# zju3dv/neuralbody

Hardware: NVIDIA H100
Metric: rays_per_s_512x512_64spp (higher is better)
Workload: dtype f16x2 (hi+lo fp16 pairs, fp32 accumulate)

## Files before the change

neuralbody_b200/csrc/nb_render_tc_list.cu:

```cuda
#include "nb_tc_common.cuh"
#include <type_traits>

namespace nb {
namespace tcl {

using tcr::Quad;

constexpr int TP = 128;
constexpr int NUM_SEGS = 6;
constexpr int MAXS = 1024;
constexpr uint32_t ID_MASK = 0x0FFFFFFFu;

__device__ __forceinline__ unsigned long long global_ns() {
    unsigned long long t;
    asm volatile("mov.u64 %0, %%globaltimer;" : "=l"(t));
    return t;
}

__device__ __forceinline__ void load_frame_xf(const RenderParams& P, FrameXf* xf, int i) {
    const int b = P.frame;
    if (i < 9) xf->R[i] = __ldg(P.R + b * 9 + i);
    if (i < 3) {
        xf->Th[i] = __ldg(P.Th + b * 3 + i);
        xf->min_dhw[i] = __ldg(P.bounds + b * 6 + (2 - i));
        xf->voxel[i] = P.voxel_size[i];
        xf->out_sh[i] = P.out_sh[i];
    }
}

constexpr int CLS_THREADS = 256, CLS_PER_THREAD = MAXS / CLS_THREADS;
__global__ void __launch_bounds__(CLS_THREADS) classify_compact_kernel(const __grid_constant__ RenderParams P) {
    __shared__ FrameXf xf;
// ... 69 lines not shown
    for (int k = 0; k < CLS_PER_THREAD; ++k) {
        const int slot = k * (CLS_THREADS / 32) + warp;
        const int c = cls[k];
        const uint32_t same = __match_any_sync(0xffffffffu, c);
        if (c >= 0) {
            int local = __popc(same & ((1u << lane) - 1));
            for (int w = 0; w < slot; ++w) local += wcnt[c][w];
            float4* buf = c >= 2 ? P.list_a : P.list_b;
            const size_t at = (c & 1) ? (size_t)sbase[c] + local : P.list_cap - (size_t)sbase[c] - stotal[c] + local;
            buf[at] = gm[k];
        } else if (live[k]) {
            P.raw_ws[(__float_as_uint(gm[k].w) & ID_MASK) - id0] = empty;
        }
    }
}

constexpr int NT = 384;
constexpr int NROWT = 96;
constexpr int LAUNCH_REGS = (65536 / NT) / 8 * 8;
constexpr int PRODUCER_REGS = 56, CONSUMER_REGS = 224;
constexpr int CHUNK_STRIDE = TP * 16 + 16;
constexpr int ACT_CHUNKS = kHidden / 8;
constexpr int PLANE_BYTES = ACT_CHUNKS * CHUNK_STRIDE;
constexpr int SEG_BUFS = 4;
constexpr int SLOT_BYTES = 16384, NUM_SLOTS = 4;
constexpr int TILE256 = kHalfTile256 * 2;
constexpr int TILE3 = kHalfTile3 * 2;
constexpr int L3_PUSH = 4;
constexpr int L3_PUSHES = (kStepsL3 + L3_PUSH - 1) / L3_PUSH;
constexpr int HEAD_FLOATS = kHidden + 4 + 3 * kColor + 4 + 3 * kHidden;
constexpr int H_ALPHA = 0, H_RGBW = kHidden + 4, H_RGBB = H_RGBW + 3 * kColor, H_B0 = H_RGBB + 4;
constexpr int OFF_HI = 0, OFF_LO = PLANE_BYTES;
constexpr int OFF_RING = 2 * PLANE_BYTES;
constexpr int OFF_HEAD = OFF_RING + NUM_SLOTS * SLOT_BYTES;
constexpr int OFF_XF = OFF_HEAD + HEAD_FLOATS * 4;
constexpr int OFF_SCHED = OFF_XF + 128;
constexpr int OFF_ROWS = OFF_SCHED + 64;
constexpr int NV_COARSE = 64, NV_FINE = 128;
__host__ __device__ constexpr int level_nv(int li) { return li < 2 ? NV_COARSE : NV_FINE; }
__host__ __device__ constexpr int level_channels(int li) { return li < 2 ? 128 : li == 2 ? 64 : 32; }
__host__ __device__ constexpr int ids_at(int li, int half) {
    return li < 2 ? (2 * li + half) * NV_COARSE : 4 * NV_COARSE + (2 * (li - 2) + half) * NV_FINE;
}
constexpr int HBITS = 8, HSIZE = 1 << HBITS;
constexpr uint32_t HEMPTY = 0xFFFFFFFFu;
struct VoxTable {
    float4 grid[TP];
// ... 266 lines not shown
                    auto put = [&](int k, float v) {
                        const __half hv = __float2half_rn(v);
                        asm volatile("st.shared.b16 [%0], %1;" ::"r"(s_lo + act_off(prow, k)), "h"(*reinterpret_cast<const unsigned short*>(&hv)) : "memory");
                    };
                    if (job < TP) {
                        positional_embed_anchored<10, 5>(e.x, e.y, e.z, [&](int j, float v) { put(j, v); });
                        put(63, 0.f);
                    } else {
                        const int smp = (int)(__float_as_uint(e.w) & ID_MASK);
                        const size_t ri = (size_t)P.frame * P.n_rays + (prow < nrows ? smp / S : 0);
                        const float dx = __ldg(P.ray_d + ri * 3), dy = __ldg(P.ray_d + ri * 3 + 1), dz = __ldg(P.ray_d + ri * 3 + 2);
                        const float nrm = sqrtf(__fadd_rn(__fadd_rn(__fmul_rn(dx, dx), __fmul_rn(dy, dy)), __fmul_rn(dz, dz)));
                        positional_embed_anchored<4, 4>(__fdiv_rn(dx, nrm), __fdiv_rn(dy, nrm), __fdiv_rn(dz, nrm), [&](int j, float v) { put(64 + j, v); });
                        put(91, 0.f); put(92, 1.f); put(93, 1.f); put(94, 0.f); put(95, 0.f);
                    }
                }
                tc::fence_proxy_async();
                tc::mbar_arrive(&bars[B_PEFULL]);
                tr.ev(32);
            }
        }
    } else {
        tc::setmaxnreg_inc<CONSUMER_REGS>();
        uint32_t s_hi, s_lo;
        const int cw = wgid - 1;
        const bool arr = lane == 0;
        int tn = ((tid & 127) == 0 && blockIdx.x == 0 && P.trace) ? (1 + cw) * 4096 : -1;
        auto tval = [&](int code, unsigned long long v) {
            if (tn >= 0 && tn < (2 + cw) * 4096) P.trace[tn++] = ((unsigned long long)code << 48) | (v & 0xFFFFFFFFFFFFull);
        };
        auto tev = [&](int code) { tval(code, (unsigned long long)clock64()); };
        const int r0 = 64 * cw + 16 * (warp & 3) + (lane >> 2), cq = 2 * (lane & 3);
        float acc0[64], acc1[64];
        auto init_bias = [&](const float* b) {
#pragma unroll
            for (int c = 0; c < 16; ++c) {
                const float2 v0 = *reinterpret_cast<const float2*>(b + 8 * c + cq), v1 = *reinterpret_cast<const float2*>(b + 128 + 8 * c + cq);
                acc0[4 * c] = v0.x; acc0[4 * c + 1] = v0.y; acc0[4 * c + 2] = v0.x; acc0[4 * c + 3] = v0.y;
                acc1[4 * c] = v1.x; acc1[4 * c + 1] = v1.y; acc1[4 * c + 2] = v1.x; acc1[4 * c + 3] = v1.y;
            }
        };
        const uint32_t wg_rows = (uint32_t)(cw * 8 * 128);
        auto mma256 = [&](uint32_t slot, int ka) {
            const uint64_t a_hi = tc::make_smem_desc(s_hi + wg_rows + 2 * ka * CHUNK_STRIDE, CHUNK_STRIDE, 128);
            const uint64_t a_lo = tc::make_smem_desc(s_lo + wg_rows + 2 * ka * CHUNK_STRIDE, CHUNK_STRIDE, 128);
            const uint64_t b0h = tc::make_smem_desc(slot + 0 * TILE256, 128 * 16, 128);
            const uint64_t b0l = tc::make_smem_desc(slot + 1 * TILE256, 128 * 16, 128);
            const uint64_t b1h = tc::make_smem_desc(slot + 2 * TILE256, 128 * 16, 128);
            const uint64_t b1l = tc::make_smem_desc(slot + 3 * TILE256, 128 * 16, 128);
            tc::wgmma_m64n128k16_f16(acc0, a_hi, b0h, true);
            tc::wgmma_m64n128k16_f16(acc1, a_hi, b1h, true);
            if (NP == 3) {
                tc::wgmma_m64n128k16_f16(acc0, a_lo, b0h, true);
                tc::wgmma_m64n128k16_f16(acc1, a_lo, b1h, true);
                tc::wgmma_m64n128k16_f16(acc0, a_hi, b0l, true);
                tc::wgmma_m64n128k16_f16(acc1, a_hi, b1l, true);
            }
        };
        uint32_t g = 0;
        uint32_t w_stall = 0, r_stall = 0, pe_stall = 0, g_coarse = 0, g_fine = 0;
        auto take = [&](auto&& mma) {
            const uint32_t s = g % NUM_SLOTS;
            const uint32_t t0 = (uint32_t)clock();
            tc::mbar_wait(&bars[B_FULL + s], (g / NUM_SLOTS) & 1);
            w_stall += (uint32_t)clock() - t0;
            tc::wgmma_fence();
            mma(s_ring + s * SLOT_BYTES);
            tc::wgmma_commit();
            ++g;
        };
        auto release = [&](uint32_t gp, bool pred) { tc::mbar_arrive_if(&bars[B_EMPTY + gp % NUM_SLOTS], pred); };
        auto release_last = [&]() { release(g - 1, arr); };

        auto convert = [&](bool last) {
            float sig0 = 0.f, sig1 = 0.f;
            auto one = [&](const float (&a)[64], int nh) {
#pragma unroll
                for (int c = 0; c < 16; ++c) {
                    const int col = 128 * nh + 8 * c + cq;
#pragma unroll
                    for (int hr = 0; hr < 2; ++hr) {
                        const float x0 = a[4 * c + 2 * hr], x1 = a[4 * c + 2 * hr + 1];
                        const uint32_t off = act_off(r0 + 8 * hr, col);
                        uint32_t hv;
                        if (last) {
                            const float2 aw = *reinterpret_cast<const float2*>(head + H_ALPHA + col);
                            float& sg = hr ? sig1 : sig0;
                            sg = fmaf(fmaxf(x0, 0.f), aw.x, sg);
                            sg = fmaf(fmaxf(x1, 0.f), aw.y, sg);
                            hv = tc::cvt_relu_f16x2(x0, x1);
                        } else if (NP == 3) {
                            hv = tc::cvt_rz_relu_f16x2(x0, x1);
                            float q0, q1;
                            tc::trunc_residual2(x0, x1, q0, q1);
                            const uint32_t lv = tc::cvt_relu_f16x2(q0, q1);
                            asm volatile("st.shared.b32 [%0], %1;" ::"r"(s_lo + off), "r"(lv) : "memory");
                        } else {
                            hv = tc::cvt_relu_f16x2(x0, x1);
                        }
                        asm volatile("st.shared.b32 [%0], %1;" ::"r"(s_hi + off), "r"(hv) : "memory");
                    }
                }
            };
            one(acc0, 0);
            one(acc1, 1);
            return make_float2(sig0, sig1);
        };
        auto publish = [&]() {
            tc::fence_proxy_async();
            tcr::named_bar_sync(1 + cw, 128);
        };

        int it = 0;
        for (int tile = blockIdx.x; tile < n_tiles; tile += gridDim.x, ++it) {
            const TileRef tref = tile_ref(tile);
            const int nrows = tref.nrows, nseg = class_segments(tref.cls);
            const float4* rows = rows_buf + (it & 1) * TP;
            asm volatile("mov.u32 %0, %1;" : "=r"(s_hi) : "r"(s_hi0));
            asm volatile("mov.u32 %0, %1;" : "=r"(s_lo) : "r"(s_lo0));
            tev(1);
            auto gather = [&](int seg) {
                const unsigned char* volbase = reinterpret_cast<const unsigned char*>(P.volume);
                const VoxTable* vt = reinterpret_cast<const VoxTable*>(smem + OFF_VTAB) + (it & 1);
                const int grp = (tid & 127) >> 3, t = tid & 7;
                const int lvl = seg < 2 ? 3 : seg < 4 ? 2 : seg < 5 ? 1 : 0;
                const int cbase0 = seg < 2 ? seg * 64 : seg < 4 ? (seg - 2) * 64 : 0;
                const int nunits = seg == NUM_SEGS - 1 ? 1 : 2;
                const int C = P.lvl_C[lvl], D = P.lvl_D[lvl], H = P.lvl_H[lvl], W = P.lvl_W[lvl];
                const int kb = 64 * (seg % SEG_BUFS);
                const int li = seg < 4 ? seg >> 1 : seg - 2;
                const int lg_vb = (li < 2 ? 7 : li == 2 ? 6 : 5) + (sizeof(VT) == 4 ? 2 : 1), lg_vpp = 10 - lg_vb;
                const bool staged = C == level_channels(li) && vt->n[2 * li + cw] <= (uint32_t)level_nv(li);
                const uint32_t st_base = s_hi + (li == 1 ? 0 : 16) * CHUNK_STRIDE + cw * 1024;
                auto stage_addr = [&](uint32_t v) {
                    const uint32_t p = v >> lg_vpp;
                    return st_base + (p >> 4) * PLANE_BYTES + (p & 15) * CHUNK_STRIDE + ((v & ((1u << lg_vpp) - 1)) << lg_vb);
                };
                if (staged && (seg >= 4 || (seg & 1) == 0)) {
                    const unsigned char* src = volbase + P.lvl_off[lvl] + (size_t)P.frame * P.lvl_bstride[lvl] * sizeof(VT);
                    const uint32_t* ids = vt->ids + ids_at(li, cw);
                    const int lg_ppv = lg_vb - 4;
                    const uint32_t nq = vt->n[2 * li + cw] << lg_ppv;
#pragma unroll 4
                    for (uint32_t i = tid & 127; i < nq; i += 128) {
                        const uint32_t v = i >> lg_ppv, q = i & ((1u << lg_ppv) - 1);
                        tc::cp_async_16(stage_addr(v) + 16 * q, src + ((size_t)ids[v] << lg_vb) + 16 * q);
                    }
                    tc::cp_async_wait_all();
                    tcr::named_bar_sync(1 + cw, 128);
                }
                auto setup = [&](float gx, float gy, float gz, float (&cw)[8]) {
                    Corners cn;
                    const uint32_t cb = clamped_cell(gx, gy, gz, W, H, D, cn);
#pragma unroll
                    for (int c = 0; c < 8; ++c) cw[c] = __fmul_rn(__fmul_rn(cn.wx[c & 1], cn.wy[(c >> 1) & 1]), cn.wz[c >> 2]);
                    return cb;
                };
                auto store_row = [&](int row, const float (&acc)[2][4]) {
#pragma unroll
                    for (int uu = 0; uu < 2; ++uu) {
                        if (uu >= nunits) continue;
                        const float (&a)[4] = acc[uu];
                        const uint32_t off = act_off(row, kb + 32 * uu + 4 * t);
                        uint2 hw, lw;
                        if (NP == 3) {
                            hw.x = tc::cvt_rz_f16x2(a[0], a[1]); hw.y = tc::cvt_rz_f16x2(a[2], a[3]);
                            float q0, q1, q2, q3;
                            tc::trunc_residual2(a[0], a[1], q0, q1);
                            tc::trunc_residual2(a[2], a[3], q2, q3);
                            lw.x = tc::cvt_f16x2(q0, q1); lw.y = tc::cvt_f16x2(q2, q3);
                            tcr::sts_v2(s_lo + off, lw);
                        } else {
                            hw.x = tc::cvt_f16x2(a[0], a[1]); hw.y = tc::cvt_f16x2(a[2], a[3]);
                        }
                        tcr::sts_v2(s_hi + off, hw);
                    }
                };
                if (staged) {
                    const uint32_t st_off = (cbase0 + 4 * t) * sizeof(VT);
#pragma unroll 1
                    for (int row = 64 * cw + grp; row < 64 * cw + 64; row += 32) {
                        float acc[2][2][4] = {};
                        float cw8[2][8];
                        uint2 sl[2];
#pragma unroll
                        for (int r = 0; r < 2; ++r) {
                            const int rw = row + 16 * r;
                            const bool occ = rw < nrows && ((__float_as_uint(rows[rw].w) >> (28 + lvl)) & 1u);
                            const float4 g = vt->grid[rw];
                            setup(g.x, g.y, g.z, cw8[r]);
                            sl[r] = *reinterpret_cast<const uint2*>(&vt->slot[rw][li][0]);
                            if (!occ) {
                                sl[r] = make_uint2(0u, 0u);
#pragma unroll
                                for (int c = 0; c < 8; ++c) cw8[r][c] = 0.f;
                            }
                        }
#pragma unroll
                        for (int c = 0; c < 8; ++c) {
                            typename Quad<VT>::raw v0[2], v1[2];
#pragma unroll
                            for (int r = 0; r < 2; ++r) {
                                const uint32_t a = stage_addr((((c < 4) ? sl[r].x : sl[r].y) >> (8 * (c & 3))) & 0xFFu) + st_off;
                                v0[r] = Quad<VT>::load_shared(a);
                                v1[r] = nunits > 1 ? Quad<VT>::load_shared(a + 32 * sizeof(VT)) : Quad<VT>::zero();
                            }
#pragma unroll
                            for (int r = 0; r < 2; ++r)
                                if (cw8[r][c] != 0.f) {
                                    Quad<VT>::fma(acc[r][0], v0[r], cw8[r][c]);
                                    Quad<VT>::fma(acc[r][1], v1[r], cw8[r][c]);
                                }
                        }
                        store_row(row, acc[0]);
                        store_row(row + 16, acc[1]);
                    }
                } else {
                    const unsigned char* lvl_ptr = volbase + P.lvl_off[lvl] + ((size_t)P.frame * P.lvl_bstride[lvl] + 4 * t) * sizeof(VT);
                    const uint32_t dX = (uint32_t)(C * sizeof(VT)), dY = dX * W, dZ = dY * H;
                    for (int row = 64 * cw + grp; row < 64 * cw + 64; row += 16) {
                        const float4 e = rows[row];
                        const bool occ = row < nrows && ((__float_as_uint(e.w) >> (28 + lvl)) & 1u);
                        float acc[2][4] = {{0.f, 0.f, 0.f, 0.f}, {0.f, 0.f, 0.f, 0.f}};
                        if (occ) {
                            float gx, gy, gz;
                            world_to_grid(*xf, e.x, e.y, e.z, gx, gy, gz);
                            float cw8[8];
                            const uint32_t cb = setup(gx, gy, gz, cw8) * dX;
#pragma unroll
                            for (int uu = 0; uu < 2; ++uu) {
                                if (uu >= nunits) continue;
                                const unsigned char* ub = lvl_ptr + (size_t)(cbase0 + 32 * uu) * sizeof(VT);
                                typename Quad<VT>::raw v[8];
#pragma unroll
                                for (int c = 0; c < 8; ++c)
                                    v[c] = Quad<VT>::load_bytes(ub + cb + ((c & 1) ? dX : 0u) + ((c & 2) ? dY : 0u) + ((c & 4) ? dZ : 0u));
#pragma unroll
                                for (int c = 0; c < 8; ++c)
                                    if (cw8[c] != 0.f) Quad<VT>::fma(acc[uu], v[c], cw8[c]);
                            }
                        }
                        store_row(row, acc);
                    }
                }
            };

            {
                const uint32_t t0 = (uint32_t)clock();
                tc::mbar_wait(&bars[B_ROWSFULL], it & 1);
                r_stall += (uint32_t)clock() - t0;
            }
            __syncwarp();
            tc::mbar_arrive_if(&bars[B_ROWSFREE], arr);
            init_bias(head + H_B0);
            for (int seg = 0; seg < nseg; ++seg) {
                const uint32_t t0 = (uint32_t)clock();
                gather(seg);
                publish();
                (seg < 4 ? g_coarse : g_fine) += (uint32_t)clock() - t0;
                const int nks = seg == NUM_SEGS - 1 ? 2 : 4, ka = 4 * (seg % SEG_BUFS);
                for (int q = 0; q < nks; ++q) {
                    take([&](uint32_t slot) { mma256(slot, ka + q); });
                    tc::wgmma_wait<1>();
                    tc::acc_fence(acc0); tc::acc_fence(acc1);
                    release(g - 2, arr && q > 0);
                }
                tc::wgmma_wait<0>();
                tc::acc_fence(acc0); tc::acc_fence(acc1);
                release_last();
            }
            tev(20);
            convert(false);
            init_bias(head + H_B0 + kHidden);
            publish();
            float2 sig = make_float2(0.f, 0.f);
            for (int layer = 1; layer <= 2; ++layer) {
                for (int q = 0; q < kKsL12; ++q) {
                    take([&](uint32_t slot) { mma256(slot, q); });
                    tc::wgmma_wait<1>();
                    tc::acc_fence(acc0); tc::acc_fence(acc1);
                    release(g - 2, arr && q > 0);
                }
                tc::wgmma_wait<0>();
                tc::acc_fence(acc0); tc::acc_fence(acc1);
                release_last();
                tev(20 + layer);
                if (layer == 1) {
                    convert(false);
                    init_bias(head + H_B0 + 2 * kHidden);
                } else {
                    tc::mbar_arrive_if(&bars[B_L2DONE], arr);
                    sig = convert(true);
                }
// ... 46 lines not shown
                }
            };
            color(c3a, 0);
            color(c3b, 1);
            float sg[2] = {sig.x, sig.y};
#pragma unroll
            for (int hr = 0; hr < 2; ++hr) {
#pragma unroll
                for (int o = 1; o <= 2; o <<= 1) {
                    cr[hr] += __shfl_xor_sync(0xffffffffu, cr[hr], o);
                    cg[hr] += __shfl_xor_sync(0xffffffffu, cg[hr], o);
                    cbl[hr] += __shfl_xor_sync(0xffffffffu, cbl[hr], o);
                    sg[hr] += __shfl_xor_sync(0xffffffffu, sg[hr], o);
                }
                const int row = r0 + 8 * hr;
                if ((lane & 3) == 0 && row < nrows) {
                    const int smp = (int)(__float_as_uint(rows[row].w) & ID_MASK);
                    P.raw_ws[smp] = make_float4(cr[hr] + head[H_RGBB], cg[hr] + head[H_RGBB + 1], cbl[hr] + head[H_RGBB + 2],
                                                sg[hr] + head[H_ALPHA + kHidden]);
                }
            }
            tev(24);
            tval(50, w_stall);
            tval(51, r_stall);
            tval(52, pe_stall);
            tval(53, g_coarse);
            tval(54, g_fine);
            w_stall = r_stall = pe_stall = g_coarse = g_fine = 0;
        }
    }
    __syncthreads();
    if (tid == 0 && P.stats) {
        atomicMax(P.frame_clock + 1, global_ns());
        const uint32_t* paths = reinterpret_cast<const uint32_t*>(smem + OFF_HCNT) + 2;
        atomicAdd(P.stats + 5, (unsigned long long)paths[0]);
        atomicAdd(P.stats + 6, (unsigned long long)paths[1]);
        atomicAdd(P.stats + 7, (unsigned long long)paths[2]);
    }
}

constexpr int COMP_WARPS = 8;
__global__ void __launch_bounds__(COMP_WARPS * 32) composite_kernel(const __grid_constant__ RenderParams P) {
    __shared__ float zs[COMP_WARPS][MAXS];
    const int warp = threadIdx.x >> 5, lane = threadIdx.x & 31;
    const int ray = blockIdx.x * COMP_WARPS + warp;
    if (blockIdx.x == 0 && threadIdx.x == 0 && P.stats) {
        const unsigned long long t0 = ~P.frame_clock[0], t1 = P.frame_clock[1];
        atomicAdd(P.stats + 2, t1 > t0 ? t1 - t0 : 0ull);
        atomicAdd(P.stats + 3, 1ull);
    }
    if (ray >= P.n_rays) return;
// ... 110 lines not shown
```

neuralbody_b200/csrc/nb_tc_common.cuh:

```cuda
#pragma once
#include "nb_device.cuh"
#include "nb_tc_ptx.cuh"

namespace nb {
namespace tcr {

__device__ __forceinline__ void named_bar_sync(int id, int nthreads) {
    asm volatile("bar.sync %0, %1;" ::"r"(id), "r"(nthreads) : "memory");
}
__device__ __forceinline__ uint4 ldg_nc_v4(const void* p) {
    uint4 r;
    asm volatile("ld.global.nc.v4.u32 {%0,%1,%2,%3}, [%4];" : "=r"(r.x), "=r"(r.y), "=r"(r.z), "=r"(r.w) : "l"(p));
    return r;
}
__device__ __forceinline__ void sts_v2(uint32_t addr, uint2 v) {
    asm volatile("st.shared.v2.b32 [%0], {%1, %2};" ::"r"(addr), "r"(v.x), "r"(v.y) : "memory");
}
__device__ __forceinline__ float f16lo_of(float x, uint32_t hi_pair, int which) {
    const __half2 h = *reinterpret_cast<const __half2*>(&hi_pair);
    return x - (which ? __high2float(h) : __low2float(h));
}

struct Tracer {
    unsigned long long* buf;
    int n;
    __device__ __forceinline__ void init(unsigned long long* base, int role) {
        buf = (base && blockIdx.x == 0) ? base + role * 4096 : nullptr;
        n = 0;
    }
    __device__ __forceinline__ void ev(int code) { val(code, (unsigned long long)clock64()); }
    __device__ __forceinline__ void val(int code, unsigned long long v) {
        if (buf && n < 4096) buf[n++] = ((unsigned long long)code << 48) | (v & 0xFFFFFFFFFFFFull);
    }
};

template <typename VT> struct Quad;
template <> struct Quad<float> {
    using raw = uint4;
    static __device__ __forceinline__ raw zero() { return make_uint4(0u, 0u, 0u, 0u); }
    static __device__ __forceinline__ raw load(const float* p) { return ldg_nc_v4(p); }
    static __device__ __forceinline__ raw load_bytes(const unsigned char* p) { return ldg_nc_v4(p); }
    static __device__ __forceinline__ raw load_shared(uint32_t addr) {
        uint4 r;
        asm volatile("ld.shared.v4.u32 {%0,%1,%2,%3}, [%4];" : "=r"(r.x), "=r"(r.y), "=r"(r.z), "=r"(r.w) : "r"(addr) : "memory");
        return r;
    }
    static __device__ __forceinline__ void fma(float (&a)[4], const raw& v, float w) {
        a[0] = fmaf(__uint_as_float(v.x), w, a[0]); a[1] = fmaf(__uint_as_float(v.y), w, a[1]);
        a[2] = fmaf(__uint_as_float(v.z), w, a[2]); a[3] = fmaf(__uint_as_float(v.w), w, a[3]);
    }
};
template <> struct Quad<__half> {
    using raw = uint2;
    static __device__ __forceinline__ raw zero() { return make_uint2(0u, 0u); }
    static __device__ __forceinline__ raw load(const __half* p) {
        uint2 r;
        asm volatile("ld.global.nc.v2.u32 {%0,%1}, [%2];" : "=r"(r.x), "=r"(r.y) : "l"(p));
        return r;
    }
    static __device__ __forceinline__ raw load_bytes(const unsigned char* p) { return load(reinterpret_cast<const __half*>(p)); }
    static __device__ __forceinline__ raw load_shared(uint32_t addr) {
        uint2 r;
        asm volatile("ld.shared.v2.u32 {%0,%1}, [%2];" : "=r"(r.x), "=r"(r.y) : "r"(addr) : "memory");
        return r;
    }
    static __device__ __forceinline__ void fma(float (&a)[4], const raw& v, float w) {
        const float2 f0 = __half22float2(*reinterpret_cast<const __half2*>(&v.x));
        const float2 f1 = __half22float2(*reinterpret_cast<const __half2*>(&v.y));
        a[0] = fmaf(f0.x, w, a[0]); a[1] = fmaf(f0.y, w, a[1]);
        a[2] = fmaf(f1.x, w, a[2]); a[3] = fmaf(f1.y, w, a[3]);
    }
};

}
}
```

neuralbody_b200/csrc/nb_tc_ptx.cuh:

```cuda
#pragma once
#include <cuda_fp16.h>
#include <stdint.h>

namespace nb {
namespace tc {

__device__ __forceinline__ uint32_t smem_u32(const void* p) { return (uint32_t)__cvta_generic_to_shared(p); }

__device__ __forceinline__ void mbar_init(uint64_t* bar, uint32_t count) {
    asm volatile("mbarrier.init.shared::cta.b64 [%0], %1;" ::"r"(smem_u32(bar)), "r"(count));
}
__device__ __forceinline__ void fence_mbar_init() { asm volatile("fence.mbarrier_init.release.cluster;" ::: "memory"); }
__device__ __forceinline__ void mbar_arrive(uint64_t* bar) {
    asm volatile("{\n\t.reg .b64 st;\n\tmbarrier.arrive.shared::cta.b64 st, [%0];\n\t}" ::"r"(smem_u32(bar)) : "memory");
}
__device__ __forceinline__ void mbar_arrive_if(uint64_t* bar, bool pred) {
    asm volatile("{\n\t.reg .pred p;\n\t.reg .b64 st;\n\tsetp.ne.b32 p, %1, 0;\n\t@p mbarrier.arrive.shared::cta.b64 st, [%0];\n\t}" ::"r"(
                     smem_u32(bar)),
                 "r"((uint32_t)pred)
                 : "memory");
}
template <int N>
__device__ __forceinline__ void setmaxnreg_dec() { asm volatile("setmaxnreg.dec.sync.aligned.u32 %0;" ::"n"(N)); }
template <int N>
// ... 41 lines not shown
}

__device__ __forceinline__ void mbar_wait_backoff(uint64_t* bar, uint32_t parity, unsigned ns) {
    uint32_t probes = 0;
    while (!mbar_try_wait(bar, parity)) {
        __nanosleep(ns);
        if (++probes > NB_WATCHDOG_PROBES * 64u) __trap();
    }
}

__device__ __forceinline__ void fence_proxy_async() { asm volatile("fence.proxy.async.shared::cta;" ::: "memory"); }

__device__ __forceinline__ void bulk_g2s(void* smem_dst, const void* gmem_src, uint32_t bytes, uint64_t* bar) {
    asm volatile("cp.async.bulk.shared::cluster.global.mbarrier::complete_tx::bytes [%0], [%1], %2, [%3];" ::"r"(
                     smem_u32(smem_dst)),
                 "l"(gmem_src), "r"(bytes), "r"(smem_u32(bar))
                 : "memory");
}

__device__ __forceinline__ void cp_async_16(uint32_t smem_dst, const void* gmem_src) {
    asm volatile("cp.async.cg.shared.global [%0], [%1], 16;" ::"r"(smem_dst), "l"(gmem_src) : "memory");
}
__device__ __forceinline__ void cp_async_wait_all() { asm volatile("cp.async.wait_all;" ::: "memory"); }

__device__ __forceinline__ uint64_t make_smem_desc(uint32_t smem_addr, uint32_t lbo_bytes, uint32_t sbo_bytes) {
    uint64_t d = 0;
    d |= (uint64_t)((smem_addr & 0x3FFFFu) >> 4);
    d |= (uint64_t)((lbo_bytes >> 4) & 0x3FFFu) << 16;
    d |= (uint64_t)((sbo_bytes >> 4) & 0x3FFFu) << 32;
    return d;
}
__device__ __forceinline__ uint64_t desc_add(uint64_t d, uint32_t bytes) { return d + (uint64_t)(bytes >> 4); }

__device__ __forceinline__ void wgmma_fence() { asm volatile("wgmma.fence.sync.aligned;" ::: "memory"); }
__device__ __forceinline__ void wgmma_commit() { asm volatile("wgmma.commit_group.sync.aligned;" ::: "memory"); }
template <int N>
__device__ __forceinline__ void wgmma_wait() { asm volatile("wgmma.wait_group.sync.aligned %0;" ::"n"(N) : "memory"); }

__device__ __forceinline__ void wgmma_m64n128k16_f16(float (&d)[64], uint64_t a_desc, uint64_t b_desc, bool accumulate) {
    asm volatile(
        "{\n\t.reg .pred p;\n\tsetp.ne.b32 p, %66, 0;\n\t"
        "wgmma.mma_async.sync.aligned.m64n128k16.f32.f16.f16 "
        "{"
        "%0,%1,%2,%3,%4,%5,%6,%7,%8,%9,%10,%11,%12,%13,%14,%15,%16,%17,%18,%19,%20,%21,%22,%23,%24,%25,%26,%2"
        "7,%28,%29,%30,%31,%32,%33,%34,%35,%36,%37,%38,%39,%40,%41,%42,%43,%44,%45,%46,%47,%48,%49,%50,%51,%5"
        "2,%53,%54,%55,%56,%57,%58,%59,%60,%61,%62,%63"
        "}, %64, %65, p, 1, 1, 0, 0;\n\t}"
        : "+f"(d[0]), "+f"(d[1]), "+f"(d[2]), "+f"(d[3]), "+f"(d[4]), "+f"(d[5]), "+f"(d[6]), "+f"(d[7]), "+f"(d[8]), "+f"(d[9]), "+f"(d[10]), "+f"(d[11]), "+f"(d[12]), "+f"(d[13]), "+f"(d[14]), "+f"(d[15]), "+f"(d[16]), "+f"(d[17]), "+f"(d[18]), "+f"(d[19]), "+f"(d[20]), "+f"(d[21]), "+f"(d[22]), "+f"(d[23]), "+f"(d[24]), "+f"(d[25]), "+f"(d[26]), "+f"(d[27]), "+f"(d[28]), "+f"(d[29]), "+f"(d[30]), "+f"(d[31]), "+f"(d[32]), "+f"(d[33]), "+f"(d[34]), "+f"(d[35]), "+f"(d[36]), "+f"(d[37]), "+f"(d[38]), "+f"(d[39]), "+f"(d[40]), "+f"(d[41]), "+f"(d[42]), "+f"(d[43]), "+f"(d[44]), "+f"(d[45]), "+f"(d[46]), "+f"(d[47]), "+f"(d[48]), "+f"(d[49]), "+f"(d[50]), "+f"(d[51]), "+f"(d[52]), "+f"(d[53]), "+f"(d[54]), "+f"(d[55]), "+f"(d[56]), "+f"(d[57]), "+f"(d[58]), "+f"(d[59]), "+f"(d[60]), "+f"(d[61]), "+f"(d[62]), "+f"(d[63])
        : "l"(a_desc), "l"(b_desc), "r"((uint32_t)accumulate)
        : "memory");
}

__device__ __forceinline__ void wgmma_m64n64k16_f16(float (&d)[32], uint64_t a_desc, uint64_t b_desc, bool accumulate) {
    asm volatile(
        "{\n\t.reg .pred p;\n\tsetp.ne.b32 p, %34, 0;\n\t"
        "wgmma.mma_async.sync.aligned.m64n64k16.f32.f16.f16 "
        "{"
        "%0,%1,%2,%3,%4,%5,%6,%7,%8,%9,%10,%11,%12,%13,%14,%15,%16,%17,%18,%19,%20,%21,%22,%23,%24,%25,%26,%2"
        "7,%28,%29,%30,%31"
        "}, %32, %33, p, 1, 1, 0, 0;\n\t}"
        : "+f"(d[0]), "+f"(d[1]), "+f"(d[2]), "+f"(d[3]), "+f"(d[4]), "+f"(d[5]), "+f"(d[6]), "+f"(d[7]), "+f"(d[8]), "+f"(d[9]), "+f"(d[10]), "+f"(d[11]), "+f"(d[12]), "+f"(d[13]), "+f"(d[14]), "+f"(d[15]), "+f"(d[16]), "+f"(d[17]), "+f"(d[18]), "+f"(d[19]), "+f"(d[20]), "+f"(d[21]), "+f"(d[22]), "+f"(d[23]), "+f"(d[24]), "+f"(d[25]), "+f"(d[26]), "+f"(d[27]), "+f"(d[28]), "+f"(d[29]), "+f"(d[30]), "+f"(d[31])
        : "l"(a_desc), "l"(b_desc), "r"((uint32_t)accumulate)
        : "memory");
}

__device__ __forceinline__ void wgmma_m64n256k8_tf32(float (&d)[128], uint64_t a_desc, uint64_t b_desc, bool accumulate) {
    asm volatile(
        "{\n\t.reg .pred p;\n\tsetp.ne.b32 p, %130, 0;\n\t"
        "wgmma.mma_async.sync.aligned.m64n256k8.f32.tf32.tf32 "
        "{"
        "%0,%1,%2,%3,%4,%5,%6,%7,%8,%9,%10,%11,%12,%13,%14,%15,%16,%17,%18,%19,%20,%21,%22,%23,%24,%25,%26,%2"
        "7,%28,%29,%30,%31,%32,%33,%34,%35,%36,%37,%38,%39,%40,%41,%42,%43,%44,%45,%46,%47,%48,%49,%50,%51,%5"
// ... 51 lines not shown
```

Before: 12.78 million.

## Feed trilinear-blended features directly into register-A wgmma per level

Replaces the segment-wise gather that wrote blended voxel features to shared-memory activation planes. The first layer now blends each 16-channel k-block in registers, splits it into hi/lo fp16 fragments and issues register-sourced wgmma directly. Voxel staging moves to per-level cp.async groups with a re-swizzled layout, and the next level's copy overlaps the current level's compute. This removes the activation-plane stores and the barrier per segment, at the cost of more register pressure and narrower 4- and 8-byte async copies and global loads.

Result: faster. 13.05 million, median of 6 (+2.2%).

```diff
diff --git a/neuralbody_b200/csrc/nb_render_tc_list.cu b/neuralbody_b200/csrc/nb_render_tc_list.cu
--- a/neuralbody_b200/csrc/nb_render_tc_list.cu
+++ b/neuralbody_b200/csrc/nb_render_tc_list.cu
@@ -7,7 +7,6 @@
 using tcr::Quad;
 
 constexpr int TP = 128;
-constexpr int NUM_SEGS = 6;
 constexpr int MAXS = 1024;
 constexpr uint32_t ID_MASK = 0x0FFFFFFFu;
 
@@ -123,7 +122,6 @@
 constexpr int CHUNK_STRIDE = TP * 16 + 16;
 constexpr int ACT_CHUNKS = kHidden / 8;
 constexpr int PLANE_BYTES = ACT_CHUNKS * CHUNK_STRIDE;
-constexpr int SEG_BUFS = 4;
 constexpr int SLOT_BYTES = 16384, NUM_SLOTS = 4;
 constexpr int TILE256 = kHalfTile256 * 2;
 constexpr int TILE3 = kHalfTile3 * 2;
@@ -436,9 +434,16 @@
         }
     } else {
         tc::setmaxnreg_inc<CONSUMER_REGS>();
+        constexpr int LG_BLK = sizeof(VT) == 4 ? 6 : 5;
+        constexpr int NCF = NP == 3 ? 2 : 4;
         uint32_t s_hi, s_lo;
         const int cw = wgid - 1;
         const bool arr = lane == 0;
+        auto wg_sync = []() {
+            uint32_t t;
+            asm volatile("mov.u32 %0, %%tid.x;" : "=r"(t));
+            tcr::named_bar_sync((int)(t >> 7), 128);
+        };
         int tn = ((tid & 127) == 0 && blockIdx.x == 0 && P.trace) ? (1 + cw) * 4096 : -1;
         auto tval = [&](int code, unsigned long long v) {
             if (tn >= 0 && tn < (2 + cw) * 4096) P.trace[tn++] = ((unsigned long long)code << 48) | (v & 0xFFFFFFFFFFFFull);
@@ -472,7 +477,7 @@
             }
         };
         uint32_t g = 0;
-        uint32_t w_stall = 0, r_stall = 0, pe_stall = 0, g_coarse = 0, g_fine = 0;
+        uint32_t w_stall = 0, pe_stall = 0, g_blend = 0, l0_wait = 0;
         auto take = [&](auto&& mma) {
             const uint32_t s = g % NUM_SLOTS;
             const uint32_t t0 = (uint32_t)clock();
@@ -488,6 +493,8 @@
 
         auto convert = [&](bool last) {
             float sig0 = 0.f, sig1 = 0.f;
+            int re;
+            asm volatile("mov.u32 %0, %1;" : "=r"(re) : "r"(r0));
             auto one = [&](const float (&a)[64], int nh) {
 #pragma unroll
                 for (int c = 0; c < 16; ++c) {
@@ -495,7 +502,7 @@
 #pragma unroll
                     for (int hr = 0; hr < 2; ++hr) {
                         const float x0 = a[4 * c + 2 * hr], x1 = a[4 * c + 2 * hr + 1];
-                        const uint32_t off = act_off(r0 + 8 * hr, col);
+                        const uint32_t off = act_off(re + 8 * hr, col);
                         uint32_t hv;
                         if (last) {
                             const float2 aw = *reinterpret_cast<const float2*>(head + H_ALPHA + col);
@@ -522,167 +529,176 @@
         };
         auto publish = [&]() {
             tc::fence_proxy_async();
-            tcr::named_bar_sync(1 + cw, 128);
+            wg_sync();
         };
 
         int it = 0;
         for (int tile = blockIdx.x; tile < n_tiles; tile += gridDim.x, ++it) {
             const TileRef tref = tile_ref(tile);
-            const int nrows = tref.nrows, nseg = class_segments(tref.cls);
+            const int nrows = tref.nrows;
             const float4* rows = rows_buf + (it & 1) * TP;
             asm volatile("mov.u32 %0, %1;" : "=r"(s_hi) : "r"(s_hi0));
             asm volatile("mov.u32 %0, %1;" : "=r"(s_lo) : "r"(s_lo0));
             tev(1);
-            auto gather = [&](int seg) {
-                const unsigned char* volbase = reinterpret_cast<const unsigned char*>(P.volume);
-                const VoxTable* vt = reinterpret_cast<const VoxTable*>(smem + OFF_VTAB) + (it & 1);
-                const int grp = (tid & 127) >> 3, t = tid & 7;
-                const int lvl = seg < 2 ? 3 : seg < 4 ? 2 : seg < 5 ? 1 : 0;
-                const int cbase0 = seg < 2 ? seg * 64 : seg < 4 ? (seg - 2) * 64 : 0;
-                const int nunits = seg == NUM_SEGS - 1 ? 1 : 2;
-                const int C = P.lvl_C[lvl], D = P.lvl_D[lvl], H = P.lvl_H[lvl], W = P.lvl_W[lvl];
-                const int kb = 64 * (seg % SEG_BUFS);
-                const int li = seg < 4 ? seg >> 1 : seg - 2;
-                const int lg_vb = (li < 2 ? 7 : li == 2 ? 6 : 5) + (sizeof(VT) == 4 ? 2 : 1), lg_vpp = 10 - lg_vb;
-                const bool staged = C == level_channels(li) && vt->n[2 * li + cw] <= (uint32_t)level_nv(li);
-                const uint32_t st_base = s_hi + (li == 1 ? 0 : 16) * CHUNK_STRIDE + cw * 1024;
-                auto stage_addr = [&](uint32_t v) {
-                    const uint32_t p = v >> lg_vpp;
-                    return st_base + (p >> 4) * PLANE_BYTES + (p & 15) * CHUNK_STRIDE + ((v & ((1u << lg_vpp) - 1)) << lg_vb);
-                };
-                if (staged && (seg >= 4 || (seg & 1) == 0)) {
+            const VoxTable* vt = reinterpret_cast<const VoxTable*>(smem + OFF_VTAB) + (it & 1);
+            const unsigned char* volbase = reinterpret_cast<const unsigned char*>(P.volume);
+            uint32_t tix;
+            asm volatile("mov.u32 %0, %%tid.x;" : "=r"(tix));
+            const int nlev = 4 - tref.cls, tq = tix & 3;
+            auto lg_vb_of = [](int li) { return (li < 2 ? 7 : li == 2 ? 6 : 5) + (sizeof(VT) == 4 ? 2 : 1); };
+            auto staged_of = [&](int li) {
+                return P.lvl_C[3 - li] == level_channels(li) && vt->n[2 * li + cw] <= (uint32_t)level_nv(li);
+            };
+            auto voxel_addr = [&](int li, uint32_t v) -> uint32_t {
+                const int lg_vb = lg_vb_of(li), lg_vpp = 10 - lg_vb;
+                const uint32_t p = v >> lg_vpp;
+                return (s_hi + ((li & 1) ? 0 : 16) * CHUNK_STRIDE + cw * 1024 + (p >> 4) * PLANE_BYTES + (p & 15) * CHUNK_STRIDE +
+                        ((v & ((1u << lg_vpp) - 1u)) << lg_vb)) >> 4;
+            };
+            auto block_addr = [](uint32_t x, uint32_t b) { return (x << 4) + (b << LG_BLK); };
+            auto stage_copy = [&](int li) {
+                if (li < nlev && staged_of(li)) {
+                    const int lvl = 3 - li, lg_vb = lg_vb_of(li), lg_ppv = lg_vb - (sizeof(VT) == 4 ? 3 : 2);
                     const unsigned char* src = volbase + P.lvl_off[lvl] + (size_t)P.frame * P.lvl_bstride[lvl] * sizeof(VT);
                     const uint32_t* ids = vt->ids + ids_at(li, cw);
-                    const int lg_ppv = lg_vb - 4;
                     const uint32_t nq = vt->n[2 * li + cw] << lg_ppv;
 #pragma unroll 4
-                    for (uint32_t i = tid & 127; i < nq; i += 128) {
-                        const uint32_t v = i >> lg_ppv, q = i & ((1u << lg_ppv) - 1);
-                        tc::cp_async_16(stage_addr(v) + 16 * q, src + ((size_t)ids[v] << lg_vb) + 16 * q);
-                    }
-                    tc::cp_async_wait_all();
-                    tcr::named_bar_sync(1 + cw, 128);
-                }
-                auto setup = [&](float gx, float gy, float gz, float (&cw)[8]) {
-                    Corners cn;
-                    const uint32_t cb = clamped_cell(gx, gy, gz, W, H, D, cn);
-#pragma unroll
-                    for (int c = 0; c < 8; ++c) cw[c] = __fmul_rn(__fmul_rn(cn.wx[c & 1], cn.wy[(c >> 1) & 1]), cn.wz[c >> 2]);
-                    return cb;
-                };
-                auto store_row = [&](int row, const float (&acc)[2][4]) {
-#pragma unroll
-                    for (int uu = 0; uu < 2; ++uu) {
-                        if (uu >= nunits) continue;
-                        const float (&a)[4] = acc[uu];
-                        const uint32_t off = act_off(row, kb + 32 * uu + 4 * t);
-                        uint2 hw, lw;
-                        if (NP == 3) {
-                            hw.x = tc::cvt_rz_f16x2(a[0], a[1]); hw.y = tc::cvt_rz_f16x2(a[2], a[3]);
-                            float q0, q1, q2, q3;
-                            tc::trunc_residual2(a[0], a[1], q0, q1);
-                            tc::trunc_residual2(a[2], a[3], q2, q3);
-                            lw.x = tc::cvt_f16x2(q0, q1); lw.y = tc::cvt_f16x2(q2, q3);
-                            tcr::sts_v2(s_lo + off, lw);
-                        } else {
-                            hw.x = tc::cvt_f16x2(a[0], a[1]); hw.y = tc::cvt_f16x2(a[2], a[3]);
-                        }
-                        tcr::sts_v2(s_hi + off, hw);
-                    }
-                };
-                if (staged) {
-                    const uint32_t st_off = (cbase0 + 4 * t) * sizeof(VT);
-#pragma unroll 1
-                    for (int row = 64 * cw + grp; row < 64 * cw + 64; row += 32) {
-                        float acc[2][2][4] = {};
-                        float cw8[2][8];
-                        uint2 sl[2];
-#pragma unroll
-                        for (int r = 0; r < 2; ++r) {
-                            const int rw = row + 16 * r;
-                            const bool occ = rw < nrows && ((__float_as_uint(rows[rw].w) >> (28 + lvl)) & 1u);
-                            const float4 g = vt->grid[rw];
-                            setup(g.x, g.y, g.z, cw8[r]);
-                            sl[r] = *reinterpret_cast<const uint2*>(&vt->slot[rw][li][0]);
-                            if (!occ) {
-                                sl[r] = make_uint2(0u, 0u);
-#pragma unroll
-                                for (int c = 0; c < 8; ++c) cw8[r][c] = 0.f;
-                            }
-                        }
-#pragma unroll
-                        for (int c = 0; c < 8; ++c) {
-                            typename Quad<VT>::raw v0[2], v1[2];
-#pragma unroll
-                            for (int r = 0; r < 2; ++r) {
-                                const uint32_t a = stage_addr((((c < 4) ? sl[r].x : sl[r].y) >> (8 * (c & 3))) & 0xFFu) + st_off;
-                                v0[r] = Quad<VT>::load_shared(a);
-                                v1[r] = nunits > 1 ? Quad<VT>::load_shared(a + 32 * sizeof(VT)) : Quad<VT>::zero();
-                            }
-#pragma unroll
-                            for (int r = 0; r < 2; ++r)
-                                if (cw8[r][c] != 0.f) {
-                                    Quad<VT>::fma(acc[r][0], v0[r], cw8[r][c]);
-                                    Quad<VT>::fma(acc[r][1], v1[r], cw8[r][c]);
-                                }
-                        }
-                        store_row(row, acc[0]);
-                        store_row(row + 16, acc[1]);
-                    }
+                    for (uint32_t i = tix & 127; i < nq; i += 128) {
+                        const uint32_t v = i >> lg_ppv, q = i & ((1u << lg_ppv) - 1u);
+                        const uint32_t dst = block_addr(voxel_addr(li, v), q >> 3) + ((q & 3u) * 4 + ((q >> 2) & 1u) * 2) * sizeof(VT);
+                        const unsigned char* s = src + ((size_t)ids[v] << lg_vb) + q * 2 * sizeof(VT);
+                        if (sizeof(VT) == 4) tc::cp_async_8(dst, s);
+                        else tc::cp_async_4(dst, s);
+                    }
+                }
+                tc::cp_async_commit();
+            };
+            auto split = [&](const float (&a)[4], int r, uint32_t (&fh)[4], uint32_t (&fl)[4]) {
+                if (NP == 3) {
+                    fh[r] = tc::cvt_rz_f16x2(a[0], a[1]); fh[2 + r] = tc::cvt_rz_f16x2(a[2], a[3]);
+                    float q0, q1, q2, q3;
+                    tc::trunc_residual2(a[0], a[1], q0, q1);
+                    tc::trunc_residual2(a[2], a[3], q2, q3);
+                    fl[r] = tc::cvt_f16x2(q0, q1); fl[2 + r] = tc::cvt_f16x2(q2, q3);
                 } else {
-                    const unsigned char* lvl_ptr = volbase + P.lvl_off[lvl] + ((size_t)P.frame * P.lvl_bstride[lvl] + 4 * t) * sizeof(VT);
-                    const uint32_t dX = (uint32_t)(C * sizeof(VT)), dY = dX * W, dZ = dY * H;
-                    for (int row = 64 * cw + grp; row < 64 * cw + 64; row += 16) {
-                        const float4 e = rows[row];
-                        const bool occ = row < nrows && ((__float_as_uint(e.w) >> (28 + lvl)) & 1u);
-                        float acc[2][4] = {{0.f, 0.f, 0.f, 0.f}, {0.f, 0.f, 0.f, 0.f}};
-                        if (occ) {
-                            float gx, gy, gz;
-                            world_to_grid(*xf, e.x, e.y, e.z, gx, gy, gz);
-                            float cw8[8];
-                            const uint32_t cb = setup(gx, gy, gz, cw8) * dX;
-#pragma unroll
-                            for (int uu = 0; uu < 2; ++uu) {
-                                if (uu >= nunits) continue;
-                                const unsigned char* ub = lvl_ptr + (size_t)(cbase0 + 32 * uu) * sizeof(VT);
-                                typename Quad<VT>::raw v[8];
-#pragma unroll
-                                for (int c = 0; c < 8; ++c)
-                                    v[c] = Quad<VT>::load_bytes(ub + cb + ((c & 1) ? dX : 0u) + ((c & 2) ? dY : 0u) + ((c & 4) ? dZ : 0u));
-#pragma unroll
-                                for (int c = 0; c < 8; ++c)
-                                    if (cw8[c] != 0.f) Quad<VT>::fma(acc[uu], v[c], cw8[c]);
-                            }
-                        }
-                        store_row(row, acc);
-                    }
+                    fh[r] = tc::cvt_f16x2(a[0], a[1]); fh[2 + r] = tc::cvt_f16x2(a[2], a[3]);
+                }
+            };
+            auto mma0 = [&](uint32_t slot, const uint32_t (&fh)[4], const uint32_t (&fl)[4]) {
+                const uint64_t b0h = tc::make_smem_desc(slot + 0 * TILE256, 128 * 16, 128);
+                const uint64_t b0l = tc::make_smem_desc(slot + 1 * TILE256, 128 * 16, 128);
+                const uint64_t b1h = tc::make_smem_desc(slot + 2 * TILE256, 128 * 16, 128);
+                const uint64_t b1l = tc::make_smem_desc(slot + 3 * TILE256, 128 * 16, 128);
+                tc::wgmma_m64n128k16_f16_ra(acc0, fh, b0h);
+                tc::wgmma_m64n128k16_f16_ra(acc1, fh, b1h);
+                if (NP == 3) {
+                    tc::wgmma_m64n128k16_f16_ra(acc0, fl, b0h);
+                    tc::wgmma_m64n128k16_f16_ra(acc1, fl, b1h);
+                    tc::wgmma_m64n128k16_f16_ra(acc0, fh, b0l);
+                    tc::wgmma_m64n128k16_f16_ra(acc1, fh, b1l);
                 }
             };
 
             {
                 const uint32_t t0 = (uint32_t)clock();
                 tc::mbar_wait(&bars[B_ROWSFULL], it & 1);
-                r_stall += (uint32_t)clock() - t0;
+                tval(51, (uint32_t)clock() - t0);
             }
             __syncwarp();
             tc::mbar_arrive_if(&bars[B_ROWSFREE], arr);
             init_bias(head + H_B0);
-            for (int seg = 0; seg < nseg; ++seg) {
+            {
                 const uint32_t t0 = (uint32_t)clock();
-                gather(seg);
-                publish();
-                (seg < 4 ? g_coarse : g_fine) += (uint32_t)clock() - t0;
-                const int nks = seg == NUM_SEGS - 1 ? 2 : 4, ka = 4 * (seg % SEG_BUFS);
-                for (int q = 0; q < nks; ++q) {
-                    take([&](uint32_t slot) { mma256(slot, ka + q); });
+                stage_copy(0);
+                stage_copy(1);
+                tc::cp_async_wait_group<1>();
+                wg_sync();
+                g_blend += (uint32_t)clock() - t0;
+            }
+            uint32_t fa_h[4], fa_l[4], fb_h[4], fb_l[4];
+#pragma unroll 1
+            for (int li = 0; li < nlev; ++li) {
+                uint32_t t0 = (uint32_t)clock();
+                if (li > 0) {
+                    tc::cp_async_wait_group<0>();
+                    wg_sync();
+                    stage_copy(li + 1);
+                }
+                const int lvl = 3 - li, D = P.lvl_D[lvl], H = P.lvl_H[lvl], W = P.lvl_W[lvl];
+                const bool staged = staged_of(li);
+                const uint32_t dX = (uint32_t)(P.lvl_C[lvl] * sizeof(VT)), dY = dX * W, dZ = dY * H;
+                float wt[2][8];
+                uint32_t va[2][4];
+#pragma unroll
+                for (int r = 0; r < 2; ++r) {
+                    const int row = r0 + 8 * r;
+                    const bool occ = row < nrows && ((__float_as_uint(rows[row].w) >> (28 + lvl)) & 1u);
+                    const float4 gq = vt->grid[row];
+                    Corners cn;
+                    const uint32_t cb = clamped_cell(gq.x, gq.y, gq.z, W, H, D, cn) * dX;
+                    const uint2 sl = *reinterpret_cast<const uint2*>(&vt->slot[row][li][0]);
+#pragma unroll
+                    for (int c = 0; c < 8; ++c) {
+                        wt[r][c] = occ ? __fmul_rn(__fmul_rn(cn.wx[c & 1], cn.wy[(c >> 1) & 1]), cn.wz[c >> 2]) : 0.f;
+                        const uint32_t s = occ ? ((((c < 4) ? sl.x : sl.y) >> (8 * (c & 3))) & 0xFFu) : 0u;
+                        if (c & 1) va[r][c >> 1] |= voxel_addr(li, s) << 16;
+                        else va[r][c >> 1] = voxel_addr(li, s);
+                    }
+                    if (!staged) va[r][0] = cb;
+                }
+                auto step = [&](auto&& blend, uint32_t b, uint32_t (&fh)[4], uint32_t (&fl)[4], bool later) {
+#pragma unroll
+                    for (int r = 0; r < 2; ++r) {
+                        float a[4] = {0.f, 0.f, 0.f, 0.f};
+#pragma unroll
+                        for (int c4 = 0; c4 < 8; c4 += NCF) {
+                            typename Quad<VT>::raw v[NCF];
+#pragma unroll
+                            for (int c = 0; c < NCF; ++c) v[c] = blend(va[r], c4 + c, b);
+#pragma unroll
+                            for (int c = 0; c < NCF; ++c)
+                                if (wt[r][c4 + c] != 0.f) Quad<VT>::fma(a, v[c], wt[r][c4 + c]);
+                        }
+                        split(a, r, fh, fl);
+                    }
+                    take([&](uint32_t slot) { mma0(slot, fh, fl); });
+                    const uint32_t t1 = (uint32_t)clock();
                     tc::wgmma_wait<1>();
+                    l0_wait += (uint32_t)clock() - t1;
                     tc::acc_fence(acc0); tc::acc_fence(acc1);
-                    release(g - 2, arr && q > 0);
-                }
+                    release(g - 2, arr && later);
+                };
+                const uint32_t nkb = (uint32_t)level_channels(li) / 16;
+                auto ksteps = [&](auto&& blend) {
+#pragma unroll 1
+                    for (uint32_t b = 0; b < nkb; b += 2) {
+                        step(blend, b, fa_h, fa_l, li > 0 || b > 0);
+                        step(blend, b + 1, fb_h, fb_l, true);
+                    }
+                };
+                if (staged) {
+                    const uint32_t tofs = 4 * tq * sizeof(VT);
+                    ksteps([&](const uint32_t (&a)[4], int c, uint32_t b) {
+                        return Quad<VT>::load_shared(block_addr((c & 1) ? a[c >> 1] >> 16 : a[c >> 1] & 0xFFFFu, b) + tofs);
+                    });
+                } else {
+                    const unsigned char* lp = volbase + P.lvl_off[lvl] + ((size_t)P.frame * P.lvl_bstride[lvl] + 2 * tq) * sizeof(VT);
+                    ksteps([&](const uint32_t (&a)[4], int c, uint32_t b) {
+                        return Quad<VT>::load_pairs(lp + a[0] + ((c & 1) ? dX : 0u) + ((c & 2) ? dY : 0u) + ((c & 4) ? dZ : 0u) +
+                                                    b * 16 * sizeof(VT));
+                    });
+                }
+                const uint32_t lcyc = (uint32_t)clock() - t0;
+                g_blend += li < 2 ? lcyc : lcyc << 16;
+            }
+            {
+                const uint32_t t0 = (uint32_t)clock();
                 tc::wgmma_wait<0>();
-                tc::acc_fence(acc0); tc::acc_fence(acc1);
-                release_last();
-            }
+                l0_wait += (uint32_t)clock() - t0;
+            }
+            tc::acc_fence(acc0); tc::acc_fence(acc1);
+            release_last();
+            wg_sync();
             tev(20);
             convert(false);
             init_bias(head + H_B0 + kHidden);
@@ -775,11 +791,11 @@
             }
             tev(24);
             tval(50, w_stall);
-            tval(51, r_stall);
             tval(52, pe_stall);
-            tval(53, g_coarse);
-            tval(54, g_fine);
-            w_stall = r_stall = pe_stall = g_coarse = g_fine = 0;
+            tval(53, g_blend & 0xFFFFu);
+            tval(54, g_blend >> 16);
+            tval(55, l0_wait);
+            w_stall = pe_stall = g_blend = l0_wait = 0;
         }
     }
     __syncthreads();
diff --git a/neuralbody_b200/csrc/nb_tc_common.cuh b/neuralbody_b200/csrc/nb_tc_common.cuh
--- a/neuralbody_b200/csrc/nb_tc_common.cuh
+++ b/neuralbody_b200/csrc/nb_tc_common.cuh
@@ -45,6 +45,12 @@
         asm volatile("ld.shared.v4.u32 {%0,%1,%2,%3}, [%4];" : "=r"(r.x), "=r"(r.y), "=r"(r.z), "=r"(r.w) : "r"(addr) : "memory");
         return r;
     }
+    static __device__ __forceinline__ raw load_pairs(const unsigned char* p) {
+        uint4 r;
+        asm volatile("ld.global.nc.v2.u32 {%0,%1}, [%2];" : "=r"(r.x), "=r"(r.y) : "l"(p));
+        asm volatile("ld.global.nc.v2.u32 {%0,%1}, [%2];" : "=r"(r.z), "=r"(r.w) : "l"(p + 32));
+        return r;
+    }
     static __device__ __forceinline__ void fma(float (&a)[4], const raw& v, float w) {
         a[0] = fmaf(__uint_as_float(v.x), w, a[0]); a[1] = fmaf(__uint_as_float(v.y), w, a[1]);
         a[2] = fmaf(__uint_as_float(v.z), w, a[2]); a[3] = fmaf(__uint_as_float(v.w), w, a[3]);
@@ -59,6 +65,12 @@
         return r;
     }
     static __device__ __forceinline__ raw load_bytes(const unsigned char* p) { return load(reinterpret_cast<const __half*>(p)); }
+    static __device__ __forceinline__ raw load_pairs(const unsigned char* p) {
+        uint2 r;
+        asm volatile("ld.global.nc.u32 %0, [%1];" : "=r"(r.x) : "l"(p));
+        asm volatile("ld.global.nc.u32 %0, [%1];" : "=r"(r.y) : "l"(p + 16));
+        return r;
+    }
     static __device__ __forceinline__ raw load_shared(uint32_t addr) {
         uint2 r;
         asm volatile("ld.shared.v2.u32 {%0,%1}, [%2];" : "=r"(r.x), "=r"(r.y) : "r"(addr) : "memory");
diff --git a/neuralbody_b200/csrc/nb_tc_ptx.cuh b/neuralbody_b200/csrc/nb_tc_ptx.cuh
--- a/neuralbody_b200/csrc/nb_tc_ptx.cuh
+++ b/neuralbody_b200/csrc/nb_tc_ptx.cuh
@@ -87,6 +87,15 @@
     asm volatile("cp.async.cg.shared.global [%0], [%1], 16;" ::"r"(smem_dst), "l"(gmem_src) : "memory");
 }
 __device__ __forceinline__ void cp_async_wait_all() { asm volatile("cp.async.wait_all;" ::: "memory"); }
+__device__ __forceinline__ void cp_async_8(uint32_t smem_dst, const void* gmem_src) {
+    asm volatile("cp.async.ca.shared.global [%0], [%1], 8;" ::"r"(smem_dst), "l"(gmem_src) : "memory");
+}
+__device__ __forceinline__ void cp_async_4(uint32_t smem_dst, const void* gmem_src) {
+    asm volatile("cp.async.ca.shared.global [%0], [%1], 4;" ::"r"(smem_dst), "l"(gmem_src) : "memory");
+}
+__device__ __forceinline__ void cp_async_commit() { asm volatile("cp.async.commit_group;" ::: "memory"); }
+template <int N>
+__device__ __forceinline__ void cp_async_wait_group() { asm volatile("cp.async.wait_group %0;" ::"n"(N) : "memory"); }
 
 __device__ __forceinline__ uint64_t make_smem_desc(uint32_t smem_addr, uint32_t lbo_bytes, uint32_t sbo_bytes) {
     uint64_t d = 0;
@@ -113,6 +122,20 @@
         "}, %64, %65, p, 1, 1, 0, 0;\n\t}"
         : "+f"(d[0]), "+f"(d[1]), "+f"(d[2]), "+f"(d[3]), "+f"(d[4]), "+f"(d[5]), "+f"(d[6]), "+f"(d[7]), "+f"(d[8]), "+f"(d[9]), "+f"(d[10]), "+f"(d[11]), "+f"(d[12]), "+f"(d[13]), "+f"(d[14]), "+f"(d[15]), "+f"(d[16]), "+f"(d[17]), "+f"(d[18]), "+f"(d[19]), "+f"(d[20]), "+f"(d[21]), "+f"(d[22]), "+f"(d[23]), "+f"(d[24]), "+f"(d[25]), "+f"(d[26]), "+f"(d[27]), "+f"(d[28]), "+f"(d[29]), "+f"(d[30]), "+f"(d[31]), "+f"(d[32]), "+f"(d[33]), "+f"(d[34]), "+f"(d[35]), "+f"(d[36]), "+f"(d[37]), "+f"(d[38]), "+f"(d[39]), "+f"(d[40]), "+f"(d[41]), "+f"(d[42]), "+f"(d[43]), "+f"(d[44]), "+f"(d[45]), "+f"(d[46]), "+f"(d[47]), "+f"(d[48]), "+f"(d[49]), "+f"(d[50]), "+f"(d[51]), "+f"(d[52]), "+f"(d[53]), "+f"(d[54]), "+f"(d[55]), "+f"(d[56]), "+f"(d[57]), "+f"(d[58]), "+f"(d[59]), "+f"(d[60]), "+f"(d[61]), "+f"(d[62]), "+f"(d[63])
         : "l"(a_desc), "l"(b_desc), "r"((uint32_t)accumulate)
+        : "memory");
+}
+
+__device__ __forceinline__ void wgmma_m64n128k16_f16_ra(float (&d)[64], const uint32_t (&a)[4], uint64_t b_desc) {
+    asm volatile(
+        "{\n\t.reg .pred p;\n\tsetp.eq.u32 p, 1, 1;\n\t"
+        "wgmma.mma_async.sync.aligned.m64n128k16.f32.f16.f16 "
+        "{"
+        "%0,%1,%2,%3,%4,%5,%6,%7,%8,%9,%10,%11,%12,%13,%14,%15,%16,%17,%18,%19,%20,%21,%22,%23,%24,%25,%26,%2"
+        "7,%28,%29,%30,%31,%32,%33,%34,%35,%36,%37,%38,%39,%40,%41,%42,%43,%44,%45,%46,%47,%48,%49,%50,%51,%5"
+        "2,%53,%54,%55,%56,%57,%58,%59,%60,%61,%62,%63"
+        "}, {%64,%65,%66,%67}, %68, p, 1, 1, 0;\n\t}"
+        : "+f"(d[0]), "+f"(d[1]), "+f"(d[2]), "+f"(d[3]), "+f"(d[4]), "+f"(d[5]), "+f"(d[6]), "+f"(d[7]), "+f"(d[8]), "+f"(d[9]), "+f"(d[10]), "+f"(d[11]), "+f"(d[12]), "+f"(d[13]), "+f"(d[14]), "+f"(d[15]), "+f"(d[16]), "+f"(d[17]), "+f"(d[18]), "+f"(d[19]), "+f"(d[20]), "+f"(d[21]), "+f"(d[22]), "+f"(d[23]), "+f"(d[24]), "+f"(d[25]), "+f"(d[26]), "+f"(d[27]), "+f"(d[28]), "+f"(d[29]), "+f"(d[30]), "+f"(d[31]), "+f"(d[32]), "+f"(d[33]), "+f"(d[34]), "+f"(d[35]), "+f"(d[36]), "+f"(d[37]), "+f"(d[38]), "+f"(d[39]), "+f"(d[40]), "+f"(d[41]), "+f"(d[42]), "+f"(d[43]), "+f"(d[44]), "+f"(d[45]), "+f"(d[46]), "+f"(d[47]), "+f"(d[48]), "+f"(d[49]), "+f"(d[50]), "+f"(d[51]), "+f"(d[52]), "+f"(d[53]), "+f"(d[54]), "+f"(d[55]), "+f"(d[56]), "+f"(d[57]), "+f"(d[58]), "+f"(d[59]), "+f"(d[60]), "+f"(d[61]), "+f"(d[62]), "+f"(d[63])
+        : "r"(a[0]), "r"(a[1]), "r"(a[2]), "r"(a[3]), "l"(b_desc)
         : "memory");
 }
 
```
